# jfjlaros/HUMID

Hardware: AMD Instinct MI355X
Metric: reads/sec deduplicated, 10M PE150 UMI=8 d=1 (higher is better)
Workload: dtype u64; 1 GPU; 10000000 reads/GPU x 1 GPU (one shuffled read set of 10000000 reads, sliced by input order), PE150 UMI=8 in header -> 24-nt packed words (8+8+8), d=1, directional clustering; synthetic molecules=N/4, family 1+Geom(3), p_sub=1e-3, p_N=1e-4; reads_per_gpu=10000000, word_nt=24, distance=1, method=directional

## Files before the change

humid_amd/_lib.py:

```python
from __future__ import annotations

import ctypes as C
import os

_HERE = os.path.dirname(os.path.abspath(__file__))
SO_PATH = os.path.join(_HERE, "libhumid_hip.so")

u64p = C.POINTER(C.c_uint64)
u32p = C.POINTER(C.c_uint32)
u8p = C.POINTER(C.c_uint8)


class HumidSummary(C.Structure):
    _fields_ = [("total", C.c_uint64), ("usable", C.c_uint64), ("unique", C.c_uint64),
                ("clusters", C.c_uint64), ("edges", C.c_uint64), ("nonsingle", C.c_uint64),
                ("ms_count", C.c_float), ("ms_neighbours", C.c_float), ("ms_cluster", C.c_float),
                ("ms_map", C.c_float), ("ms_total", C.c_float), ("ms_h2d", C.c_float),
                ("ms_d2h", C.c_float), ("ms_k_insert", C.c_float), ("ms_k_pairs", C.c_float),
                ("ms_k_cluster", C.c_float), ("ms_k_map", C.c_float), ("ms_k_part", C.c_float),
                ("ms_k_unperm", C.c_float), ("count_mode_used", C.c_uint32)]

    def asdict(self):
        d = {k: getattr(self, k) for k, _ in self._fields_}
        d["records8"] = bool(d["count_mode_used"] >> 8)
# ... 208 lines not shown
    "humid_stage_count": (C.c_int, [C.c_void_p, C.c_void_p, C.c_void_p, C.c_uint64, C.c_uint32,
                                    C.c_uint64, C.c_uint64, C.c_uint64, u64p, u64p]),
    "humid_stage_unique": (C.c_int, [C.c_void_p, C.POINTER(C.c_void_p), C.POINTER(C.c_void_p),
                                     C.POINTER(C.c_void_p)]),
    "humid_stage_graph": (C.c_int, [C.c_void_p, C.c_void_p, C.c_void_p, C.c_uint64, C.c_uint32,
                                    C.c_uint32, C.c_uint32, C.POINTER(C.c_void_p),
                                    C.POINTER(C.c_void_p), C.POINTER(HumidSummary)]),
    "humid_stage_map": (C.c_int, [C.c_void_p, C.c_void_p, C.c_void_p, C.c_uint64, C.c_void_p,
                                  C.c_void_p]),
    "humid_stage_count_dense": (C.c_int, [C.c_void_p, C.c_void_p, C.c_void_p, C.c_uint64, C.c_uint32,
                                          C.c_uint64, C.c_uint64, u64p, C.c_uint32, u64p, u64p, u64p]),
    "humid_stage_map_dense": (C.c_int, [C.c_void_p, C.c_void_p, C.c_void_p, C.POINTER(C.c_void_p), u64p]),
    "humid_stage_pairs": (C.c_int, [C.c_void_p, C.c_void_p, C.c_uint64, C.c_uint32, C.c_uint32,
                                    C.c_uint32, C.c_uint32, C.POINTER(C.c_void_p), u64p]),
    "humid_graph_split_info": (C.c_int, [C.c_void_p, C.POINTER(C.c_uint64), C.POINTER(C.c_uint64), u32p]),
    "humid_get_run_roads": (C.c_int, [C.c_void_p, C.POINTER(HumidRunRoads)]),
    "humid_stage_kernel_ms": (C.c_int, [C.c_void_p, C.POINTER(C.c_float), C.POINTER(C.c_float), u32p]),
    "humid_stage_route_words": (C.c_int, [C.c_void_p, C.c_void_p, C.c_uint64, C.POINTER(C.c_void_p)]),
    "humid_stage_route": (C.c_int, [C.c_void_p, C.c_void_p, C.c_void_p, C.c_uint64, u64p, u64p, C.c_uint32, u64p,
                                    C.POINTER(C.c_void_p), C.POINTER(C.c_void_p)]),
    "humid_stage_route_check": (C.c_int, [C.c_void_p]),
    "humid_stage_exchange_ids": (C.c_int, [C.c_void_p, C.c_void_p, C.c_void_p, C.c_void_p, C.c_uint64,
                                           C.c_uint64, C.c_uint64, C.c_uint64, C.POINTER(C.c_void_p),
                                           C.POINTER(C.c_void_p)]),
    "humid_stage_plan_info": (C.c_int, [C.c_void_p, C.c_uint32, C.c_uint32, C.c_uint64, u32p, u32p]),
    "humid_stage_combo_route": (C.c_int, [C.c_void_p, C.c_void_p, C.c_void_p, C.c_uint64, C.c_uint64,
                                          C.c_uint32, C.c_uint32, C.c_uint64, C.c_uint32, C.c_uint32,
                                          C.POINTER(C.c_void_p), u64p]),
    "humid_stage_pairs_keyed": (C.c_int, [C.c_void_p, C.c_void_p, C.c_uint64, C.c_int, C.c_uint64,
                                          C.c_void_p, C.c_uint32, C.c_uint32, C.c_uint64, C.c_uint32,
# ... 66 lines not shown
```

humid_amd/api.py:

```python
from __future__ import annotations

import ctypes as C

import numpy as np

from . import _lib

DIRECTIONAL = 0
MAXIMUM = 1

BEST_LEAF, BEST_CLUSTER = 0, 1
NO_READ = 0xffffffff
NO_TILE = 0xffffffff
_BEST_SCOPES = {"leaf": BEST_LEAF, "cluster": BEST_CLUSTER, BEST_LEAF: BEST_LEAF, BEST_CLUSTER: BEST_CLUSTER}

STRAND_TOP, STRAND_BOTTOM, STRAND_NONE = 0, 1, 2

BC_FILTERED, BC_EXACT, BC_CORRECTED, BC_AMBIGUOUS, BC_UNMATCHED = range(5)

CELLS_TOP, CELLS_EXPECTED, CELLS_MIN_READS = 0, 1, 2


class HumidError(RuntimeError):
    def __init__(self, code, msg):
# ... 616 lines not shown
        self._check(self._lib.humid_get_leaves(self._h, _vp(out["word"]), _vp(out["count"]),
                                               _vp(out["first_read"]), _vp(out["degree"]),
                                               _vp(out["cluster_id"]), _vp(out["is_max_leaf"])))
        if getattr(self, "_grouped_summary", None) is self.summary:
            out["group"] = np.zeros(u, np.uint32)
            self._check(self._lib.humid_get_leaf_groups(self._h, _vp(out["group"])))
        if getattr(self, "_keyed_summary", None) is self.summary:
            out["key"] = self.group_keys()[out["group"]] if u else np.zeros(0, np.uint64)
        return out

    def graph_split_info(self):
        a, b, f = C.c_uint64(), C.c_uint64(), C.c_uint32()
        self._check(self._lib.humid_graph_split_info(self._h, C.byref(a), C.byref(b), C.byref(f)))
        return dict(pairs_direct=a.value, pairs_graph=b.value, full_graph_built=f.value)

    def run_roads(self):
        r = _lib.HumidRunRoads()
        self._check(self._lib.humid_get_run_roads(self._h, C.byref(r)))
        return r.asdict()

    def adjacency(self):
        u = int(self.summary["unique"])
        e2 = 2 * int(self.summary["edges"])
        off = np.zeros(u + 1, np.uint32)
        idx = np.zeros(max(e2, 1), np.uint32)
        self._check(self._lib.humid_get_adjacency(self._h, _vp(off), _vp(idx)))
        return off, idx[:e2]

    def clusters(self):
        c = int(self.summary["clusters"])
# ... 218 lines not shown
```

humid_amd/csrc/humid_hip.hip:

```cpp
#include "pipeline.hip.h"
#include "passes.hip.h"

static std::string g_err;
extern "C" __attribute__((visibility("hidden"))) void humid_set_global_error(const char *text) { g_err = text ? text : ""; }

extern "C" {

uint32_t humid_abi_version(void) { return HUMID_ABI_VERSION; }

int humid_device_count(void) {
  int n = 0;
  if (hipGetDeviceCount(&n) != hipSuccess) return 0;
  return n;
}

const char *humid_last_error(const humid_ctx *ctx) { return ctx ? ctx->err.c_str() : g_err.c_str(); }

int humid_ctx_create(humid_ctx **out, int device, void *stream) {
  humid_ctx *c = nullptr;
  if (!out) return fail(nullptr, HUMID_E_INVALID, "out is null");
  *out = nullptr;
  int ndev = 0;
  hipError_t e = hipGetDeviceCount(&ndev);
  if (e != hipSuccess || ndev == 0)
// ... 142 lines not shown
  }
  if (strcmp(key, "compact_graph") == 0) {
    c->use_compact = value != 0;
    return HUMID_OK;
  }
  if (strcmp(key, "group_buckets") == 0) {
    c->group_buckets = value != 0;
    return HUMID_OK;
  }
  if (strcmp(key, "fused_search") == 0) {
    c->fused_search = value != 0;
    return HUMID_OK;
  }
  if (strcmp(key, "pair_split") == 0) {
    c->pair_split = value != 0;
    return HUMID_OK;
  }
  if (strcmp(key, "padded_partition") == 0) {
    c->pt_padded = value != 0;
    return HUMID_OK;
  }
  if (strcmp(key, "force_comm") == 0) {
    c->force_comm = value != 0;
    return HUMID_OK;
  }
  if (strcmp(key, "bucket_walk") == 0) {
    if (value < 0 || value > (1 << 24)) return fail(c, HUMID_E_INVALID, "bucket_walk must be 0 (no limit) .. 2^24");
    c->walk_max = (u32)value;
    return HUMID_OK;
  }
// ... 231 lines not shown
#define NEED_LEAVES()                                                                         \
  do {                                                                                        \
    if (!c) return fail(nullptr, HUMID_E_INVALID, "ctx is null");                             \
    if (!state_has_leaves(c)) return fail(c, HUMID_E_STATE, "no completed dedup run / graph stage in this context"); \
    HIPCHK(hipSetDevice(c->device));                                                          \
    TRY(expand_compact(c));                                                                   \
  } while (0)

int humid_graph_split_info(humid_ctx *c, uint64_t *pairs_direct, uint64_t *pairs_graph, uint32_t *full_graph_built) {
  if (!c) return fail(nullptr, HUMID_E_INVALID, "ctx is null");
  if (!state_has_leaves(c)) return fail(c, HUMID_E_STATE, "no completed dedup run / graph stage in this context");
  const bool split = c->cg_valid && c->cg_split;
  if (pairs_direct) *pairs_direct = split ? c->cg_iso : 0;
  if (pairs_graph) *pairs_graph = split ? c->cg_R : c->E;
  if (full_graph_built) *full_graph_built = (!split || c->cg_full) ? 1u : 0u;
  return HUMID_OK;
}

int humid_get_run_roads(humid_ctx *c, humid_run_roads *out) {
  if (!c) return fail(nullptr, HUMID_E_INVALID, "ctx is null");
  if (!out) return fail(c, HUMID_E_INVALID, "null argument");
  if (c->state.holds == CtxState::NOTHING) return fail(c, HUMID_E_STATE, "no completed run or stage call in this context");
  *out = c->roads;
  return HUMID_OK;
}

int humid_get_leaves(humid_ctx *c, uint64_t *word, uint32_t *count, uint32_t *first_read,
                     uint32_t *degree, uint32_t *cluster_id, uint8_t *is_max_leaf) {
  NEED_LEAVES();
  size_t U = (size_t)c->gU;
// ... 1167 lines not shown
```

humid_amd/csrc/kernels_cgraph.hip.h:

```cpp
#ifndef HUMID_KERNELS_CGRAPH_HIP_H
#define HUMID_KERNELS_CGRAPH_HIP_H

#include "common.hip.h"
#include "kernels_graph.hip.h"
#include "kernels_cluster.hip.h"

#define ER_REGIONS 64u
#define ER_STRIDE 32u
struct EdgeRegs {
  u64 *e;
  u32 cap_r;
  u32 *cur;
  const u64 *far;
  u32 n_far;
};
__device__ __forceinline__ u32 er_count(const EdgeRegs &er, u32 r) {
  if (r == ER_REGIONS) return er.n_far;
  const u32 c = er.cur[r * ER_STRIDE];
  return c < er.cap_r ? c : er.cap_r;
}
__device__ __forceinline__ u64 *er_at(const EdgeRegs &er, u32 r, u32 k) {
  return r == ER_REGIONS ? (u64 *)er.far + k : er.e + (size_t)r * er.cap_r + k;
}

// ... 190 lines not shown
  if (PASS0) pa_emit<PA_PPT, 4, MULTI>(word, IdxSelf{}, i0, 256u, n, found, first_off, rule, er, bits, multi, overflow, lds);
  else pa_emit<PA_PPT, 4, MULTI>(word, IdxGlobal{V}, i0, 256u, n, found, first_off, rule, er, bits, multi, overflow, lds);
  PH(2); PH(3); PH(4);
  PH_END(5, 4, (blockIdx.x & 15u) == 5u);
}

struct WordsLds {
  const u64 *sw;
  __device__ __forceinline__ u64 operator()(u32 j) const { return sw[j]; }
};
struct IdxGrouped {
  const unsigned short *inv;
  const u32 *v_in;
  __device__ __forceinline__ u32 operator()(u32 j) const { return v_in[inv[j]]; }
};
template <bool MULTI>
struct PairSearchDevT {
  static constexpr bool on = true;
  PairRule<u64> rule;
  EdgeRegs er;
  u32 *bits;
  u32 *multi;
  ull *big;
  u32 *overflow;
  template <u32 NP, u32 T>
  __device__ __forceinline__ void in_bin(const u64 *sw, u32 n, const unsigned short *inv, const u32 *v_in, u32 *scratch) const {
    const WordsLds word{sw};
    u32 found[NP], first_off[NP];
#pragma unroll
    for (u32 q = 0; q < NP; q++) {
      const u32 i = threadIdx.x + q * T;
      found[q] = 0; first_off[q] = 0;
      if (i < n) pa_walk(word, sw[i], sw[i + 1 < n ? i + 1 : i], i, n, rule, big, found[q], first_off[q]);
    }
    pa_emit<NP, T / 64u, MULTI>(word, IdxGrouped{inv, v_in}, threadIdx.x, T, n, found, first_off, rule, er, bits, multi, overflow, scratch);
  }
};

using PairSearchDev = PairSearchDevT<false>;

static __global__ void __launch_bounds__(256)
k_mark_pairs(const u64 *__restrict__ pairs, u32 n_pairs, u32 n_leaves, u32 *bits, u32 *bad, u32 *multi = nullptr) {
  HUMID_GUARD_LAST_VGPR();
  const u32 k = blockIdx.x * blockDim.x + threadIdx.x;
  if (k >= n_pairs) return;
  const u64 e = pairs[k];
  const u32 a = (u32)(e >> 32), b = (u32)e;
  if (a >= n_leaves || b >= n_leaves || a == b) { *bad = 1; return; }
  if (multi) { mark_end<true>(bits, multi, a); mark_end<true>(bits, multi, b); }
  else { mark_end<false>(bits, multi, a); mark_end<false>(bits, multi, b); }
// ... 343 lines not shown
```

humid_amd/csrc/kernels_graph.hip.h:

```cpp
#ifndef HUMID_KERNELS_GRAPH_HIP_H
#define HUMID_KERNELS_GRAPH_HIP_H

#include "common.hip.h"

#define MAX_COMBOS 20
#define MAX_FIELDS 8
struct ComboPlan {
  u32 ncombo;
  u32 key_bits;
  W2 mask[MAX_COMBOS];
  u8 nfield[MAX_COMBOS];
  u8 shift[MAX_COMBOS][MAX_FIELDS];
  u8 width[MAX_COMBOS][MAX_FIELDS];
};

template <class WT>
struct EarlierMasksT {
  WT m[MAX_COMBOS];
};

struct ComboFields {
  u32 nf;
  u8 shift[MAX_FIELDS];
  u8 width[MAX_FIELDS];
// ... 42 lines not shown
  u32 kb;
  __device__ __forceinline__ bool load(u32 j, u64 &payload) const {
    const W2 w = words[j];
    u64 k = 0;
#pragma unroll
    for (u32 f = 0; f < MAX_FIELDS; f++) {
      if (f < cf.nf) {
        const u32 wd = cf.width[f];
        k = ((wd >= 64) ? 0ull : (k << wd)) | w_field(w, cf.shift[f], wd);
      }
    }
    payload = k << (64 - kb);
    return true;
  }
  __device__ __forceinline__ u64 key(u64 payload) const { return payload; }
};

__device__ __forceinline__ u32 uf_find(const u32 *P, u32 x) {
  u32 p = ld_agent(&P[x]);
  while (p != x) { x = p; p = ld_agent(&P[x]); }
  return x;
}

__device__ __forceinline__ void uf_union(u32 *P, u32 a, u32 b) {
  while (true) {
    a = uf_find(P, a);
    b = uf_find(P, b);
    if (a == b) return;
    if (a > b) { u32 t = a; a = b; b = t; }
    if (atomicCAS(&P[b], b, a) == b) return;
// ... 613 lines not shown
```

humid_amd/csrc/kernels_part.hip.h:

```cpp
#ifndef HUMID_KERNELS_PART_HIP_H
#define HUMID_KERNELS_PART_HIP_H

#include "common.hip.h"
#include "kernels_count.hip.h"

#define PT_THREADS 1024u
#define PT_TILE 8192u
#define PT_IPT (PT_TILE / PT_THREADS)
#define PT_MAXBINS 512u
#define PT_MAXBINS1 1024u

struct PtInput {
  const u64 *words;
  const u8 *filtered;
  u64 rlo, rhi;
  u32 check_range;
  PartKeyOp key;
};
__device__ __forceinline__ bool pt_load(const PtInput &in, u32 r, u64 &key) {
  if (in.filtered && in.filtered[r]) return false;
  const u64 w = in.words[r];
  if (in.check_range && (w < in.rlo || w > in.rhi)) return false;
  key = in.key(w);
  return true;
// ... 219 lines not shown
  for (u32 b = threadIdx.x; b < nb; b += PT_THREADS) h[b] = 0;
  __syncthreads();
  const u32 beg = s_beg, n = s_cnt;
  for (u32 j = threadIdx.x; j < n; j += PT_THREADS)
    atomicAdd(&h[(u32)(src.key(k_in[beg + j]) >> (64 - d1 - d2)) & (nb - 1)], 1u);
  __syncthreads();
  for (u32 b = threadIdx.x; b < nb; b += PT_THREADS)
    if (h[b]) atomicAdd(&hist_fine[(s_c << d2) | b], h[b]);
}

struct NoSearch { static constexpr bool on = false; };
#define GF_THREADS 1024u
#define GF_MAXBITS 15u
#define GF_SMALL 7872u
#define GF_MID 32768u
template <class SRC, int SIZE, class SEARCH = NoSearch>
__global__ void __launch_bounds__(GF_THREADS, SIZE == 0 ? 8 : 4)
k_group_fine(SRC src, const u64 *__restrict__ k_in, const u32 *__restrict__ v_in, const u32 *__restrict__ cbase, u32 d1,
             u32 d2, u64 *__restrict__ k_out, u32 *__restrict__ v_out, u32 cap1, SEARCH srch = SEARCH()) {
  HUMID_GUARD_LAST_VGPR();
  static_assert(SIZE == 0 || !SEARCH::on, "the search rides in the launch of the small bins");
  static_assert(GF_SMALL * 2u + 32u <= (1u << (GF_MAXBITS - 1)), "the grouped words and the emit's words fit the counter area");
  constexpr bool BIG = SIZE == 2;
  constexpr u32 INV_WORDS = SIZE == 0 ? GF_SMALL / 2u + 16u : (1u << (GF_MAXBITS - 1)) + 16u;
  __shared__ __attribute__((aligned(8))) u32 gf_lds[BIG ? (1u << GF_MAXBITS) + 16 : (1u << (GF_MAXBITS - 1)) + INV_WORDS];
  const u32 nb = 1u << d2, c = blockIdx.x;
  PH_DECL;
  PH(0);
  const u32 beg = cbase[c], end = cbase[c + 1];
  if (beg >= end) return;
// ... 23 lines not shown
#pragma unroll
      for (u32 q = 0; q < GF_RPT; q++) {
        const u32 j = threadIdx.x + q * GF_THREADS;
        ff[q] = fine(kk[q]);
        if (j < n) atomicAdd(&gf_lds[ff[q] >> 1], 1u << (16 * (ff[q] & 1)));
      }
    } else {
      for (u32 j = threadIdx.x; j < n; j += GF_THREADS) {
        const u32 f = fine(k_in[j]);
        atomicAdd(&gf_lds[f >> 1], 1u << (16 * (f & 1)));
      }
    }
    PH(2);
    __syncthreads();
    PH(3);
    const u32 words = nb >= 2 ? nb / 2 : 1u;
    const u32 n_waves = GF_THREADS / 64u;
    const u32 per_wave = (words + n_waves - 1) / n_waves, wbeg = wv * per_wave, wend = wbeg + per_wave < words ? wbeg + per_wave : words;
    u32 tot = 0;
    for (u32 w = wbeg + lane; w < wend; w += 64) { const u32 x = gf_lds[w]; tot += (x & 0xffffu) + (x >> 16); }
#pragma unroll
    for (u32 dd = 32; dd; dd >>= 1) tot += __shfl_xor(tot, dd);
    if (lane == 0) wsum[wv] = tot;
    __syncthreads();
    u32 run = 0;
    for (u32 q = 0; q < wv; q++) run += wsum[q];
    for (u32 w0 = wbeg; w0 < wend; w0 += 64) {
      const u32 w = w0 + lane;
      const u32 x = w < wend ? gf_lds[w] : 0u;
      const u32 mine = (x & 0xffffu) + (x >> 16);
      const u32 incl = wave_incl_scan(mine);
      const u32 lo = run + incl - mine, hi = lo + (x & 0xffffu);
      if (w < wend) gf_lds[w] = lo | (hi << 16);
      run += (u32)__builtin_amdgcn_readlane((int)incl, 63);
    }
    __syncthreads();
    PH(4);
    if constexpr (SIZE == 0) {
      u32 oldq[GF_RPT];
#pragma unroll
      for (u32 q = 0; q < GF_RPT; q++) {
        const u32 j = threadIdx.x + q * GF_THREADS;
        oldq[q] = j < n ? atomicAdd(&gf_lds[ff[q] >> 1], 1u << (16 * (ff[q] & 1))) : 0u;
      }
#pragma unroll
      for (u32 q = 0; q < GF_RPT; q++) {
        const u32 j = threadIdx.x + q * GF_THREADS;
        if (j < n) inv[(oldq[q] >> (16 * (ff[q] & 1))) & 0xffffu] = (unsigned short)j;
      }
      PH(5);
      __syncthreads();
// ... 58 lines not shown
  u32 run = incl - mine;
  for (u32 q = 0; q < wv; q++) run += wsum[q];
  if (b0 < nb)
    for (u32 q = 0; q < per; q++) {
      const u32 x = gf_lds[b0 + q];
      gf_lds[b0 + q] = run;
      run += x;
    }
  __syncthreads();
  for (u32 j = threadIdx.x; j < n; j += GF_THREADS) {
    const u64 w = k_in[j];
    const u32 p = atomicAdd(&gf_lds[fine(w)], 1u);
    k_out[p] = w;
    v_out[p] = v_in[j];
  }
}

#define UW_MAXBINS 2048u
#define UW_MAXSHIFT 15u

static __global__ void __launch_bounds__(1024)
k_unperm_bins(const u32 *__restrict__ vals, const u32 *__restrict__ pslot, const u64 *__restrict__ slot_out,
              const u32 *__restrict__ n_pos_dev, u32 n_pos_max, u32 n_reads, u32 wshift, u32 n_bins, u32 *ucur,
              u64 *__restrict__ rec) {
  HUMID_GUARD_LAST_VGPR();
  __shared__ u64 srec[PT_TILE];
  __shared__ unsigned short sbin[PT_TILE];
  __shared__ u32 cnt[UW_MAXBINS], loff[UW_MAXBINS + 1], goff[UW_MAXBINS], wsum[16];
  u32 n_pos = n_pos_dev ? *n_pos_dev : n_pos_max;
  if (n_pos > n_pos_max) n_pos = n_pos_max;
// ... 114 lines not shown
```

humid_amd/csrc/kernels_part8.hip.h:

```cpp
#ifndef HUMID_KERNELS_PART8_HIP_H
#define HUMID_KERNELS_PART8_HIP_H

#include "common.hip.h"
#include "kernels_count.hip.h"
#include "kernels_part.hip.h"

#define P8_CAP2_LOG 10u
#define P8_CAP2 (1u << P8_CAP2_LOG)
#define P8_RPT (P8_CAP2 / 256u)

struct RecKey {
  u64 lo, scale;
  u32 z, kbits;
  u32 pow2;
  __host__ __device__ __forceinline__ u64 operator()(u64 w) const { return ((w - lo) * scale) >> z; }
  __device__ __forceinline__ u64 word(u64 k) const {
    if (pow2) return lo + k;
    const u64 x = k << z, q = x / scale;
    return lo + q + ((x - q * scale) ? 1u : 0u);
  }
};

struct Reads8 {
  const u64 *words;
// ... 18 lines not shown
    const u32 bin = b0 + sub;
    if (bin >= nb) continue;
    const u32 beg = loff[bin], n = loff[bin + 1] - beg;
    for (u32 k = gl; k < n; k += G) {
      const u64 d = dst(bin, k);
      if (d != ~0ull) out[d] = srec[beg + k];
    }
  }
}
__device__ __forceinline__ u32 p8_group(u32 records, u32 nb) {
  u32 g = 8;
  while (g < 64 && g * nb < records) g <<= 1;
  return g;
}

template <class SRC, u32 THREADS>
__global__ void __launch_bounds__(THREADS)
k_p8_scatter1(SRC src, u32 n_reads, u32 kbits, u32 d1, u32 ibits, u32 cap1, u32 *cursor, u64 *__restrict__ out, ull *ctr) {
  HUMID_GUARD_LAST_VGPR();
  constexpr u32 TILE = THREADS * PT_IPT;
  __shared__ u64 srec[TILE];
  __shared__ u32 cnt[PT_MAXBINS1], loff[PT_MAXBINS1 + 1], goff[PT_MAXBINS1], wsum[16];
  const u32 nb = 1u << d1;
  PH_DECL;
  PH(0);
  const u32 t_beg = blockIdx.x * TILE;
  const u32 t_cnt = (t_beg >= n_reads) ? 0u : ((n_reads - t_beg < TILE) ? n_reads - t_beg : TILE);
  for (u32 b = threadIdx.x; b < nb; b += THREADS) cnt[b] = 0;
  __syncthreads();
  PH(1);
  const u32 rbits = kbits - d1;
// ... 7 lines not shown
    if (j < t_cnt && src.load(t_beg + j, k)) {
      const u32 bin = (u32)(k >> rbits);
      rec[q] = ((k & ((1ull << rbits) - 1ull)) << ibits) | (u64)(t_beg + j);
      binrank[q] = bin << 16 | atomicAdd(&cnt[bin], 1u);
    }
  }
  PH(2);
  __syncthreads();
  PH(3);
  block_exscan_1024(cnt, loff, nb, wsum);
  PH(4);
  if (threadIdx.x < nb) {
    const u32 c = cnt[threadIdx.x];
    const u32 had = c ? atomicAdd(&cursor[threadIdx.x], c) : 0u;
    goff[threadIdx.x] = threadIdx.x * cap1 + (had < cap1 ? had : cap1);
    if (had + c > cap1) ctr[CTR_SPECIAL] = 1;
  }
  PH(5);
#pragma unroll
  for (u32 q = 0; q < PT_IPT; q++)
    if (binrank[q] != NONE32) srec[loff[binrank[q] >> 16] + (binrank[q] & 0xffffu)] = rec[q];
  __syncthreads();
  PH(6);
  p8_write_bins(srec, loff, nb, p8_group(loff[nb], nb), out,
                [&](u32 bin, u32 k) -> u64 { return goff[bin] + k < (bin + 1) * cap1 ? (u64)goff[bin] + k : ~0ull; });
  PH(7);
  PH_END(1, 7, (blockIdx.x & 15u) == 3u);
}

static __global__ void __launch_bounds__(1024, 8)
k_p8_scatter2(const u64 *__restrict__ in, const u32 *__restrict__ tprefix, const u32 *__restrict__ cbase, u32 kbits, u32 d1,
// ... 552 lines not shown
```

humid_amd/csrc/pipeline.hip.h:

```cpp
#ifndef HUMID_PIPELINE_HIP_H
#define HUMID_PIPELINE_HIP_H

#include <fcntl.h>
#include <sys/mman.h>
#include <sys/stat.h>
#include <unistd.h>

#include <atomic>
#include <cerrno>
#include <chrono>
#include <type_traits>
#include <utility>

#include "common.hip.h"
#include "prims.hip.h"
#include "kernels_count.hip.h"
#include "kernels_part.hip.h"
#include "kernels_part8.hip.h"
#include "kernels_graph.hip.h"
#include "kernels_cluster.hip.h"
#include "kernels_cgraph.hip.h"
#include "kernels_map.hip.h"
#include "kernels_xchg.hip.h"
#include "kernels_wide.hip.h"
// ... 125 lines not shown
  u64 cg_pairs_bound = 0;
  u32 cg_method = 0;
  const u32 *ctr_x[3] = {nullptr, nullptr, nullptr};
  DBuf xo_gw, xo_gc;
  DBuf xo_regs, xo_inv;
  u64 xr_ecap = 0;
  DBuf xo_send, xo_int, xo_cross, xo_sel, xo_selall, xo_parent, xo_flag, xo_xroot, xo_xcbits, xo_xcblk, xo_xcid, xo_xcall, xo_ldeg, xo_cnt;
  DBuf pw_a, pw_ai, pw_b, pw_bi;
  DBuf p8_a, p8_b, p8_cur, p8_status;
  bool use_rec8 = true;
  bool last_rec8 = false;
  const u32 *rec_cursor2 = nullptr;
  DBuf pt_work, unperm_rec, route_tiles;
  bool group_buckets = true;
  bool fused_search = true;
  bool pt_padded = true;
  bool use_tile_partition = true;
  bool last_part_tiled = false;
  int x_test_fail_after = -1, x_gathers = 0;
  bool x_hist_done = false, x_peer_failed = false;
  bool route_checked = true;
  const u32 *route_bad = nullptr;
  bool last_unperm_tiled = false;
  bool oc_valid = false, oc_fits = false;
  u32 oc_n = 0, oc_nt = 0;
  u64 oc_lo = 0, oc_scale = 0;
  u32 n_parts = 0;
  bool stage_map_timed = false;
  bool last_count_sorted = false;
  u32 g_wpr = 1;
// ... 1009 lines not shown
  if (n_runs) HIPCHK(hipMemcpy(d_runs, runs.data(), (size_t)n_runs * sizeof(BigRun), hipMemcpyHostToDevice));
  *d_runs_out = d_runs;
  return HUMID_OK;
}

static ComboFields plan_fields(const ComboPlan &plan, u32 cb) {
  ComboFields cf;
  cf.nf = plan.nfield[cb];
  for (u32 f = 0; f < MAX_FIELDS; f++) { cf.shift[f] = plan.shift[cb][f]; cf.width[f] = plan.width[cb][f]; }
  return cf;
}
struct GroupRide {
  PairSearchDev group;
  bool did_group = false;
  hipEvent_t ev_group[2] = {nullptr, nullptr};
};
static void group_fine_with_search(humid_ctx *c, const FieldsSrc &src, const u64 *k0, const u32 *v0, const u32 *cbase, u32 d1, u32 d2, u64 *ws,
                                   u32 *vs, u32 cap1, const PairSearchDev &s);
template <class SRC, class WT>
static int group_words_by_stretch(humid_ctx *c, const ComboPlan &plan, u32 cb, const WT *W, u32 n, u64 *ws, u32 *vs, bool *done,
                                  bool may_pad = false, GroupRide *ride = nullptr) {
  hipStream_t st = c->stream;
  u32 bit_n = 0;
  for (u32 f = 0; f < plan.nfield[cb]; f++) bit_n += plan.width[cb][f];
  *done = c->group_buckets && plan.nfield[cb] >= 1 && bit_n >= 2 && bit_n <= 24 && n >= 4096;
  c->gf_valid = nullptr;
  if (!*done) return HUMID_OK;
  const u32 d1 = bit_n >= 18 ? 9u : (bit_n + 1) / 2, d2 = bit_n - d1;
  const u32 nb1 = 1u << d1;
  const bool padded = may_pad && c->gf_padded;
  const u32 cap1 = padded ? n / nb1 + n / nb1 / 4 + 1024 : 0u;
  const size_t room = padded ? (size_t)nb1 * cap1 : (size_t)n;
  ENSURE(c->pt_work, (size_t)(1024 + 513 + 513 + 516) * 4);
  u32 *hist1 = c->pt_work.as<u32>(), *cursor1 = hist1 + 512, *cbase = cursor1 + 512, *tprefix = cbase + 513, *dummy = tprefix + 513;
  if (padded) {
    if (!c->gf_cur.p) {
      ENSURE(c->gf_cur, 512 * 4);
      HIPCHK(hipMemsetAsync(c->gf_cur.p, 0, 512 * 4, st));
    }
    cursor1 = c->gf_cur.as<u32>();
  } else HIPCHK(hipMemsetAsync(c->pt_work.p, 0, 1024 * 4, st));
  ENSURE(c->seg_k0, room * 8);
  ENSURE(c->seg_v0, room * 4);
  const SRC src{W, plan_fields(plan, cb), bit_n};
  const u32 tiles1 = (n + PT_TILE - 1) / PT_TILE;
  if (!padded) {
    hipLaunchKernelGGL(k_pt_hist1<SRC>, dim3(tiles1 < 512 ? tiles1 : 512), dim3(1024), 0, st, src, n, d1, hist1);
    hipLaunchKernelGGL(k_pt_scan1, dim3(1), dim3(1024), 0, st, (const u32 *)hist1, d1, 0u, cbase, tprefix, dummy, dummy + 513, 0u);
  }
  static const bool gs_small = getenv("HUMID_GS_THREADS") ? atoi(getenv("HUMID_GS_THREADS")) == 512 : false;
  const bool ride_ok = ride && std::is_same<SRC, FieldsSrc>::value && padded && cap1 <= GF_SMALL;
  if (gs_small)
    hipLaunchKernelGGL((k_pt_scatter<1, SRC, 512>), dim3((n + 4095) / 4096), dim3(512), 0, st, src, n, (const u64 *)nullptr,
                       (const u32 *)nullptr, (const u32 *)nullptr, (const u32 *)nullptr, d1, d2, (const u32 *)cbase, cursor1,
                       c->seg_k0.as<u64>(), c->seg_v0.as<u32>(), (u32 *)nullptr, cap1, &c->d_ctr[CTR_GOVER]);
  else
    hipLaunchKernelGGL((k_pt_scatter<1, SRC>), dim3(tiles1), dim3(1024), 0, st, src, n, (const u64 *)nullptr,
                       (const u32 *)nullptr, (const u32 *)nullptr, (const u32 *)nullptr, d1, d2, (const u32 *)cbase, cursor1,
                       c->seg_k0.as<u64>(), c->seg_v0.as<u32>(), (u32 *)nullptr, cap1, &c->d_ctr[CTR_GOVER]);
  if (padded)
    hipLaunchKernelGGL(k_pt_scan1, dim3(1), dim3(1024), 0, st, (const u32 *)cursor1, d1, 0u, cbase, tprefix, dummy, dummy + 513, cap1, cursor1);
  c->gf_valid = padded ? (const u32 *)(cbase + nb1) : (const u32 *)nullptr;
  const u32 largest = padded ? cap1 : n;
  if (ride_ok) {
    if constexpr (std::is_same<SRC, FieldsSrc>::value) {
      if (ride->ev_group[0]) HIPCHK(hipEventRecord(ride->ev_group[0], st));
// ... 166 lines not shown
  else
    hipLaunchKernelGGL((k_pairs_append<true, WT>), grid, blk, 0, c->stream, w.W, w.V, w.n, rule, er, bits, multi, big, overflow, n_valid);
}
static PairSearchDev pairs_append_dev(const PairSearch<u64> &s, u64 mask, u32 cb, const EdgeRegs &er, u32 *bits, u32 *multi, ull *big,
                                      u32 *overflow) {
  return PairSearchDev{PairRule<u64>{mask, s.em, cb, s.distance, s.walk_max}, er, bits, multi, big, overflow};
}
static void group_fine_with_search(humid_ctx *c, const FieldsSrc &src, const u64 *k0, const u32 *v0, const u32 *cbase, u32 d1, u32 d2, u64 *ws,
                                   u32 *vs, u32 cap1, const PairSearchDev &s) {
  if (s.multi)
    hipLaunchKernelGGL((k_group_fine<FieldsSrc, 0, PairSearchDevT<true>>), dim3(1u << d1), dim3(GF_THREADS), 0, c->stream, src, k0, v0, cbase, d1, d2,
                       ws, vs, cap1, PairSearchDevT<true>{s.rule, s.er, s.bits, s.multi, s.big, s.overflow});
  else
    hipLaunchKernelGGL((k_group_fine<FieldsSrc, 0, PairSearchDev>), dim3(1u << d1), dim3(GF_THREADS), 0, c->stream, src, k0, v0, cbase, d1, d2, ws,
                       vs, cap1, s);
}
static void comp_stats(humid_ctx *c, u32 U) {
  hipLaunchKernelGGL(k_comp_stats, dim3(blocks_for(U)), dim3(256), 0, c->stream, c->deg.as<u32>(), c->parent.as<u32>(), U, c->csize.as<u32>());
  hipLaunchKernelGGL(k_comp_count, dim3(512), dim3(256), 0, c->stream, c->deg.as<u32>(), c->parent.as<u32>(), c->csize.as<u32>(), U, c->d_ctr,
                     c->small_roots.as<u32>());
}

template <class WT>
static int stage_graph(humid_ctx *c, const WT *g_word, const u32 *g_cnt, u32 U, u32 word_nt,
                       u32 distance, u32 method, humid_summary &s, u32 &n_pair_segs_out,
                       const u64 *ext_edges = nullptr, u64 n_ext_edges = 0) {
  hipStream_t st = c->stream;
  c->g_word = g_word;
  c->g_wpr = (u32)(sizeof(WT) / 8);
  c->g_cnt = g_cnt;
// ... 227 lines not shown
}

template <class WT>
static int stage_graph_compact(humid_ctx *c, const WT *g_word, const u32 *g_cnt, u32 U, u32 word_nt,
                               u32 distance, u32 method, humid_summary &s, u32 &n_pair_segs_out,
                               const u64 *ext_edges = nullptr, u64 n_ext_edges = 0) {
  hipStream_t st = c->stream;
  c->g_word = g_word;
  c->g_wpr = (u32)(sizeof(WT) / 8);
  c->g_cnt = g_cnt;
  c->gU = U;
  c->cg_valid = false;
  c->cg_expanded = false;
  c->cg_split = c->cg_full = c->cg_m_late = c->cg_broken = false;
  c->cg_iso = c->cg_R = 0;
  const bool split = c->pair_split;
  const ComboPlan plan = make_plan(word_nt - c->gk_nt, distance, U, c->force_segments, true, c->gk_nt);
  const PairSearch<WT> ps = pair_search<WT>(c, plan, distance);
  const bool given = ext_edges != nullptr;
  const bool search = !given && distance > 0 && U > 1;
  if (search && plan.ncombo == 1 && plan.key_bits == 0 && U > (1u << 18))
    return fail(c, HUMID_E_OVERFLOW, "distance %u over %u-nt words compares all pairs of %u unique words: too many neighbour pairs",
                distance, word_nt, U);
  if (given && n_ext_edges > 0x7fffffffull) return fail(c, HUMID_E_OVERFLOW, "too many neighbour pairs");
  const u32 nseg = search ? plan.ncombo : 0;
  const u32 n_words = (((U + 31) / 32) + 7) & ~7u, n_blk = n_words / 8;
  c->cg_nblocks = n_blk;
  ENSURE(c->cg_bits, (size_t)n_words * 4);
  ENSURE(c->cg_nbits, (size_t)n_words * 4);
  ENSURE(c->cg_blk, ((size_t)n_blk + 1) * 4);
// ... 39 lines not shown
      if (split) {
        z.p[4] = multi; z.n[4] = n_words;
        z.p[5] = c->cg_rbits.as<u32>(); z.n[5] = n_words;
        z.p[6] = c->small.as<u32>(); z.n[6] = SPLIT_WORDS;
      }
      hipLaunchKernelGGL(k_zero_many, dim3(64), dim3(256), 0, st, z);
    }
    auto search_alone = [&](u32 seg) -> int {
      if (seg < 8 && c->kev_on) HIPCHK(hipEventRecord(c->kev[20 + 2 * seg], st));
      pairs_append<WT>(c, ps, walked_seg<WT>(c, plan, seg, g_word, U), er, c->cg_bits.as<u32>(), multi, &c->d_ctr[CTR_BIGMASK],
                       (u32 *)&c->d_ctr[CTR_EOVER], seg_valid[seg]);
      if (seg < 8 && c->kev_on) HIPCHK(hipEventRecord(c->kev[21 + 2 * seg], st));
      return HUMID_OK;
    };
    const bool ride_on = c->fused_search && std::is_same<WT, u64>::value;
    for (u32 seg = 0; seg < nseg; seg++) {
      bool searched = false;
      if (seg) {
        seg_valid[seg] = nullptr;
        if (!ordered_seg[seg]) {
          GroupRide ride;
          if constexpr (std::is_same<WT, u64>::value) {
            if (ride_on) {
              ride.group = pairs_append_dev(ps, w_from<u64>(plan.mask[seg]), seg, er, c->cg_bits.as<u32>(), multi, &c->d_ctr[CTR_BIGMASK], (u32 *)&c->d_ctr[CTR_EOVER]);
              if (seg < 8 && c->kev_on) { ride.ev_group[0] = c->kev[20 + 2 * seg]; ride.ev_group[1] = c->kev[21 + 2 * seg]; }
            }
          }
          TRY(bucket_order<WT>(c, plan, seg, g_word, U, seg_ws<WT>(c, seg, U), seg_vs(c, seg, U), true, ride_on ? &ride : nullptr));
          seg_valid[seg] = c->gf_valid;
          searched = ride.did_group;
        }
        ordered_seg[seg] = true;
      }
      if (!searched) TRY(search_alone(seg));
    }
    if (n_far)
      hipLaunchKernelGGL(k_mark_pairs, dim3(blocks_for(n_far)), dim3(256), 0, st, far, (u32)n_far, U, c->cg_bits.as<u32>(), bad, multi);
    if (split) {
      const u64 rest_cap = (u64)ER_REGIONS * er.cap_r + n_far;
      if (rest_cap > 0x7fffffffull) return fail(c, HUMID_E_OVERFLOW, "too many neighbour pairs");
      ENSURE(c->cg_rest, (size_t)(rest_cap + 1) * 8);
      const u32 gx = (u32)std::min<u64>(std::max<u64>(blocks_for(std::max<u64>(er.cap_r, er.n_far), SPLIT_PPT * 256), 1), 4096);
      u32 *sp = c->small.as<u32>();
      if (method == HUMID_METHOD_MAXIMUM)
        hipLaunchKernelGGL(k_pairs_split<true>, dim3(gx, ER_REGIONS + 1), dim3(256), 0, st, er, (const u32 *)multi, g_cnt, c->cg_pres.as<u32>(),
                           c->cg_nbits.as<u32>(), c->cg_rbits.as<u32>(), c->cg_rest.as<u64>(), (u32)rest_cap, U, sp);
      else
// ... 29 lines not shown
      continue;
    }
    if (given) {
      u32 h_bad = 0;
      HIPCHK(hipMemcpyAsync(&h_bad, bad, 4, hipMemcpyDeviceToHost, st));
      HIPCHK(hipStreamSynchronize(st));
      if (h_bad) return fail(c, HUMID_E_INVALID, "malformed edge list (node index out of range)");
    }
    if (search && cgs.big_mask && !far) {
      const u64 big_mask = cgs.big_mask;
      u64 got = 0;
      for (int phase = 0; phase < 2; phase++) {
        u64 at = 0;
        for (u32 seg = 0; seg < nseg; seg++) {
          if (!(big_mask >> seg & 1)) continue;
          const Walked<WT> w = walked_seg<WT>(c, plan, seg, g_word, U);
          std::vector<BigRun> runs;
          const BigRun *d_runs = nullptr;
          TRY(find_big_runs<WT>(c, w.W, U, w.mask, ps.walk_max, seg, runs, &d_runs));
          if (!runs.back().tile0) continue;
          const ull start = phase ? at : 0;
          HIPCHK(hipMemcpyAsync(&c->d_ctr[CTR_SPECIAL], &start, sizeof(ull), hipMemcpyHostToDevice, st));
          HIPCHK(hipStreamSynchronize(st));
          tiles_emit<WT>(c, ps, w, d_runs, runs, phase ? PM_EMIT_FILL : PM_EMIT_COUNT,
                         EmitSink{nullptr, nullptr, c->cg_far.as<u64>(), &c->d_ctr[CTR_SPECIAL]});
          HIPCHK(hipGetLastError());
          TRY(read_counters(c));
          if (phase == 0) got += c->h_ctr[CTR_SPECIAL]; else at = c->h_ctr[CTR_SPECIAL];
        }
        if (phase == 0) {
// ... 1239 lines not shown
```

include/humid_hip.h:

```cpp
#ifndef HUMID_HIP_H
#define HUMID_HIP_H

#include <stddef.h>
#include <stdint.h>

#ifdef __cplusplus
extern "C" {
#endif

#define HUMID_OK             0
#define HUMID_E_INVALID     -1
#define HUMID_E_UNSUPPORTED -2
#define HUMID_E_NOMEM       -3
#define HUMID_E_HIP         -4
#define HUMID_E_OVERFLOW    -5
#define HUMID_E_STATE       -6

#define HUMID_METHOD_DIRECTIONAL 0u
#define HUMID_METHOD_MAXIMUM     1u

#define HUMID_ABI_VERSION 5u

typedef struct humid_ctx humid_ctx;

// ... 318 lines not shown
                             const uint64_t **d_unique_edges, uint64_t *n_unique_edges);

int humid_stage_owned_results(humid_ctx *ctx, const uint32_t *d_local_cluster_id,
                              const uint8_t *d_local_is_max, const uint64_t *shard_begin,
                              uint32_t n_shards, const uint32_t **d_packed, uint64_t *counts);
int humid_stage_owner_perm(humid_ctx *ctx, const uint64_t *d_words, const uint8_t *d_filtered,
                           uint64_t n_reads, const uint64_t *range_lo, const uint64_t *range_hi,
                           uint32_t n_ranks, const uint32_t **d_perm, uint64_t *counts);
int humid_stage_owner_perm_wide(humid_ctx *ctx, const uint64_t *d_words, const uint8_t *d_filtered,
                                uint64_t n_reads, uint32_t word_nt, const uint64_t *range_lo, const uint64_t *range_hi,
                                uint32_t n_ranks, const uint32_t **d_perm, uint64_t *counts);
int humid_stage_scatter(humid_ctx *ctx, const uint32_t *d_perm, const uint32_t *d_packed,
                        uint64_t n_recv, uint64_t n_reads, uint32_t *d_cluster_id, uint8_t *d_keep);

int humid_graph_split_info(humid_ctx *ctx, uint64_t *pairs_direct, uint64_t *pairs_graph, uint32_t *full_graph_built);
#define HUMID_ROAD_PART_PADDED_REDO 1
#define HUMID_ROAD_ORDERS_REDONE    2
#define HUMID_ROAD_REGIONS_REGROWN  3
#define HUMID_ROAD_FAR_TILES        4
#define HUMID_ROAD_CSR_TILES        5
#define HUMID_ROAD_JOIN_PIECES      6
#define HUMID_ROADS_MAX 32
typedef struct humid_run_roads {
  uint32_t n_events;
  uint32_t graph_attempts;
  uint8_t events[HUMID_ROADS_MAX];
} humid_run_roads;
int humid_get_run_roads(humid_ctx *ctx, humid_run_roads *out);
int humid_stage_kernel_ms(humid_ctx *ctx, float *ms_k_insert, float *ms_k_map, uint32_t *count_mode_used);
int humid_stage_route_words(humid_ctx *ctx, const uint64_t *d_words, uint64_t n_send,
// ... 58 lines not shown
```

Baseline: 17.72 billion reads/s.

## Search neighbour pairs on packed records and skip storing segment orders

```diff
diff --git a/humid_amd/_lib.py b/humid_amd/_lib.py
--- a/humid_amd/_lib.py
+++ b/humid_amd/_lib.py
@@ -246,6 +246,7 @@
     "humid_stage_pairs": (C.c_int, [C.c_void_p, C.c_void_p, C.c_uint64, C.c_uint32, C.c_uint32,
                                     C.c_uint32, C.c_uint32, C.POINTER(C.c_void_p), u64p]),
     "humid_graph_split_info": (C.c_int, [C.c_void_p, C.POINTER(C.c_uint64), C.POINTER(C.c_uint64), u32p]),
+    "humid_group_records_info": (C.c_int, [C.c_void_p, u32p, u32p]),
     "humid_get_run_roads": (C.c_int, [C.c_void_p, C.POINTER(HumidRunRoads)]),
     "humid_stage_kernel_ms": (C.c_int, [C.c_void_p, C.POINTER(C.c_float), C.POINTER(C.c_float), u32p]),
     "humid_stage_route_words": (C.c_int, [C.c_void_p, C.c_void_p, C.c_uint64, C.POINTER(C.c_void_p)]),
diff --git a/humid_amd/api.py b/humid_amd/api.py
--- a/humid_amd/api.py
+++ b/humid_amd/api.py
@@ -654,6 +654,11 @@
         self._check(self._lib.humid_graph_split_info(self._h, C.byref(a), C.byref(b), C.byref(f)))
         return dict(pairs_direct=a.value, pairs_graph=b.value, full_graph_built=f.value)
 
+    def group_records_info(self):
+        a, b = C.c_uint32(), C.c_uint32()
+        self._check(self._lib.humid_group_records_info(self._h, C.byref(a), C.byref(b)))
+        return dict(searched_on_records=a.value, orders_stored=b.value)
+
     def run_roads(self):
         r = _lib.HumidRunRoads()
         self._check(self._lib.humid_get_run_roads(self._h, C.byref(r)))
diff --git a/humid_amd/csrc/humid_hip.hip b/humid_amd/csrc/humid_hip.hip
--- a/humid_amd/csrc/humid_hip.hip
+++ b/humid_amd/csrc/humid_hip.hip
@@ -180,6 +180,10 @@
   }
   if (strcmp(key, "pair_split") == 0) {
     c->pair_split = value != 0;
+    return HUMID_OK;
+  }
+  if (strcmp(key, "group_records") == 0) {
+    c->group_records = value != 0;
     return HUMID_OK;
   }
   if (strcmp(key, "padded_partition") == 0) {
@@ -441,6 +445,14 @@
   if (pairs_direct) *pairs_direct = split ? c->cg_iso : 0;
   if (pairs_graph) *pairs_graph = split ? c->cg_R : c->E;
   if (full_graph_built) *full_graph_built = (!split || c->cg_full) ? 1u : 0u;
+  return HUMID_OK;
+}
+
+int humid_group_records_info(humid_ctx *c, uint32_t *searched_on_records, uint32_t *orders_stored) {
+  if (!c) return fail(nullptr, HUMID_E_INVALID, "ctx is null");
+  if (!state_has_leaves(c)) return fail(c, HUMID_E_STATE, "no completed dedup run / graph stage in this context");
+  if (searched_on_records) *searched_on_records = c->cg_valid ? c->gr_rides : 0u;
+  if (orders_stored) *orders_stored = c->cg_valid ? c->gr_orders : 0u;
   return HUMID_OK;
 }
 
diff --git a/humid_amd/csrc/kernels_cgraph.hip.h b/humid_amd/csrc/kernels_cgraph.hip.h
--- a/humid_amd/csrc/kernels_cgraph.hip.h
+++ b/humid_amd/csrc/kernels_cgraph.hip.h
@@ -228,6 +228,12 @@
   const u32 *v_in;
   __device__ __forceinline__ u32 operator()(u32 j) const { return v_in[inv[j]]; }
 };
+struct IdxRecords {
+  const unsigned short *inv;
+  const u64 *recs;
+  u32 ibits;
+  __device__ __forceinline__ u32 operator()(u32 j) const { return (u32)(recs[inv[j]] & ((1ull << ibits) - 1ull)); }
+};
 template <bool MULTI>
 struct PairSearchDevT {
   static constexpr bool on = true;
@@ -239,6 +245,14 @@
   u32 *overflow;
   template <u32 NP, u32 T>
   __device__ __forceinline__ void in_bin(const u64 *sw, u32 n, const unsigned short *inv, const u32 *v_in, u32 *scratch) const {
+    walk_bin<NP, T>(sw, n, IdxGrouped{inv, v_in}, scratch);
+  }
+  template <u32 NP, u32 T>
+  __device__ __forceinline__ void in_bin_recs(const u64 *sw, u32 n, const unsigned short *inv, const u64 *recs, u32 ibits, u32 *scratch) const {
+    walk_bin<NP, T>(sw, n, IdxRecords{inv, recs, ibits}, scratch);
+  }
+  template <u32 NP, u32 T, class IDX>
+  __device__ __forceinline__ void walk_bin(const u64 *sw, u32 n, const IDX &idx, u32 *scratch) const {
     const WordsLds word{sw};
     u32 found[NP], first_off[NP];
 #pragma unroll
@@ -247,7 +261,7 @@
       found[q] = 0; first_off[q] = 0;
       if (i < n) pa_walk(word, sw[i], sw[i + 1 < n ? i + 1 : i], i, n, rule, big, found[q], first_off[q]);
     }
-    pa_emit<NP, T / 64u, MULTI>(word, IdxGrouped{inv, v_in}, threadIdx.x, T, n, found, first_off, rule, er, bits, multi, overflow, scratch);
+    pa_emit<NP, T / 64u, MULTI>(word, idx, threadIdx.x, T, n, found, first_off, rule, er, bits, multi, overflow, scratch);
   }
 };
 
diff --git a/humid_amd/csrc/kernels_graph.hip.h b/humid_amd/csrc/kernels_graph.hip.h
--- a/humid_amd/csrc/kernels_graph.hip.h
+++ b/humid_amd/csrc/kernels_graph.hip.h
@@ -80,6 +80,24 @@
     return true;
   }
   __device__ __forceinline__ u64 key(u64 payload) const { return payload; }
+};
+
+struct RecSqueeze {
+  u32 p, d1;
+  __device__ __forceinline__ u64 low(u64 x) const { return x & ((1ull << p) - 1ull); }
+  __device__ __forceinline__ u32 bin(u64 w) const { return (u32)(w >> p) & ((1u << d1) - 1u); }
+  __device__ __forceinline__ u64 squeeze(u64 w) const { return (w >> p >> d1 << p) | low(w); }
+  __device__ __forceinline__ u64 word(u32 c, u64 s) const { return (s >> p << p << d1) | ((u64)c << p) | low(s); }
+};
+struct FieldsRecs {
+  const u64 *words;
+  RecSqueeze sq;
+  u32 rbits;
+  __device__ __forceinline__ bool load(u32 j, u64 &k) const {
+    const u64 w = words[j];
+    k = ((u64)sq.bin(w) << rbits) | (sq.squeeze(w) & ((1ull << rbits) - 1ull));
+    return true;
+  }
 };
 
 __device__ __forceinline__ u32 uf_find(const u32 *P, u32 x) {
diff --git a/humid_amd/csrc/kernels_part.hip.h b/humid_amd/csrc/kernels_part.hip.h
--- a/humid_amd/csrc/kernels_part.hip.h
+++ b/humid_amd/csrc/kernels_part.hip.h
@@ -257,6 +257,31 @@
 #define GF_MAXBITS 15u
 #define GF_SMALL 7872u
 #define GF_MID 32768u
+__device__ __forceinline__ void gf_scan16(u32 *cnt, u32 *wsum, u32 nb) {
+  const u32 lane = threadIdx.x & 63, wv = threadIdx.x >> 6;
+  const u32 words = nb >= 2 ? nb / 2 : 1u;
+  const u32 n_waves = GF_THREADS / 64u;
+  const u32 per_wave = (words + n_waves - 1) / n_waves, wbeg = wv * per_wave, wend = wbeg + per_wave < words ? wbeg + per_wave : words;
+  u32 tot = 0;
+  for (u32 w = wbeg + lane; w < wend; w += 64) { const u32 x = cnt[w]; tot += (x & 0xffffu) + (x >> 16); }
+#pragma unroll
+  for (u32 dd = 32; dd; dd >>= 1) tot += __shfl_xor(tot, dd);
+  if (lane == 0) wsum[wv] = tot;
+  __syncthreads();
+  u32 run = 0;
+  for (u32 q = 0; q < wv; q++) run += wsum[q];
+  for (u32 w0 = wbeg; w0 < wend; w0 += 64) {
+    const u32 w = w0 + lane;
+    const u32 x = w < wend ? cnt[w] : 0u;
+    const u32 mine = (x & 0xffffu) + (x >> 16);
+    const u32 incl = wave_incl_scan(mine);
+    const u32 lo = run + incl - mine, hi = lo + (x & 0xffffu);
+    if (w < wend) cnt[w] = lo | (hi << 16);
+    run += (u32)__builtin_amdgcn_readlane((int)incl, 63);
+  }
+  __syncthreads();
+}
+
 template <class SRC, int SIZE, class SEARCH = NoSearch>
 __global__ void __launch_bounds__(GF_THREADS, SIZE == 0 ? 8 : 4)
 k_group_fine(SRC src, const u64 *__restrict__ k_in, const u32 *__restrict__ v_in, const u32 *__restrict__ cbase, u32 d1,
@@ -310,27 +335,7 @@
     PH(2);
     __syncthreads();
     PH(3);
-    const u32 words = nb >= 2 ? nb / 2 : 1u;
-    const u32 n_waves = GF_THREADS / 64u;
-    const u32 per_wave = (words + n_waves - 1) / n_waves, wbeg = wv * per_wave, wend = wbeg + per_wave < words ? wbeg + per_wave : words;
-    u32 tot = 0;
-    for (u32 w = wbeg + lane; w < wend; w += 64) { const u32 x = gf_lds[w]; tot += (x & 0xffffu) + (x >> 16); }
-#pragma unroll
-    for (u32 dd = 32; dd; dd >>= 1) tot += __shfl_xor(tot, dd);
-    if (lane == 0) wsum[wv] = tot;
-    __syncthreads();
-    u32 run = 0;
-    for (u32 q = 0; q < wv; q++) run += wsum[q];
-    for (u32 w0 = wbeg; w0 < wend; w0 += 64) {
-      const u32 w = w0 + lane;
-      const u32 x = w < wend ? gf_lds[w] : 0u;
-      const u32 mine = (x & 0xffffu) + (x >> 16);
-      const u32 incl = wave_incl_scan(mine);
-      const u32 lo = run + incl - mine, hi = lo + (x & 0xffffu);
-      if (w < wend) gf_lds[w] = lo | (hi << 16);
-      run += (u32)__builtin_amdgcn_readlane((int)incl, 63);
-    }
-    __syncthreads();
+    gf_scan16(gf_lds, wsum, nb);
     PH(4);
     if constexpr (SIZE == 0) {
       u32 oldq[GF_RPT];
@@ -419,6 +424,65 @@
     k_out[p] = w;
     v_out[p] = v_in[j];
   }
+}
+
+template <class SRC, class SQ, class SEARCH>
+__global__ void __launch_bounds__(GF_THREADS, 8)
+k_group_fine_recs(SRC src, SQ sq, const u64 *__restrict__ recs, u32 *cursor, u32 d1, u32 d2, u32 ibits, u32 cap1, SEARCH srch) {
+  HUMID_GUARD_LAST_VGPR();
+  constexpr u32 INV_WORDS = GF_SMALL / 2u + 16u;
+  constexpr u32 GF_RPT = 8;
+  static_assert(GF_RPT * GF_THREADS >= GF_SMALL, "a thread holds its share of a full bin");
+  static_assert(GF_SMALL * 2u + 32u <= (1u << (GF_MAXBITS - 1)), "the grouped words and the emit's words fit the counter area");
+  __shared__ __attribute__((aligned(8))) u32 gf_lds[(1u << (GF_MAXBITS - 1)) + INV_WORDS];
+  const u32 nb = 1u << d2, c = blockIdx.x;
+  u32 n = cursor[c];
+  if (n == 0) return;
+  if (n > cap1) n = cap1;
+  if (n > GF_SMALL) n = GF_SMALL;
+  recs += (size_t)c * cap1;
+  u32 *wsum = gf_lds + (1u << (GF_MAXBITS - 1)) + INV_WORDS - 16;
+  unsigned short *inv = (unsigned short *)(gf_lds + (1u << (GF_MAXBITS - 1)));
+  u64 kk[GF_RPT];
+  u32 ff[GF_RPT];
+#pragma unroll
+  for (u32 q = 0; q < GF_RPT; q++) {
+    const u32 j = threadIdx.x + q * GF_THREADS;
+    kk[q] = j < n ? recs[j] : 0ull;
+  }
+  for (u32 b = threadIdx.x; b < (1u << (GF_MAXBITS - 1)); b += GF_THREADS) gf_lds[b] = 0;
+  __syncthreads();
+  if (threadIdx.x == 0) cursor[c] = 0;
+#pragma unroll
+  for (u32 q = 0; q < GF_RPT; q++) {
+    const u32 j = threadIdx.x + q * GF_THREADS;
+    kk[q] = sq.word(c, kk[q] >> ibits);
+    ff[q] = (u32)(src.key(kk[q]) >> (64 - d1 - d2)) & (nb - 1);
+    if (j < n) atomicAdd(&gf_lds[ff[q] >> 1], 1u << (16 * (ff[q] & 1)));
+  }
+  __syncthreads();
+  gf_scan16(gf_lds, wsum, nb);
+  u32 oldq[GF_RPT];
+#pragma unroll
+  for (u32 q = 0; q < GF_RPT; q++) {
+    const u32 j = threadIdx.x + q * GF_THREADS;
+    oldq[q] = j < n ? atomicAdd(&gf_lds[ff[q] >> 1], 1u << (16 * (ff[q] & 1))) : 0u;
+  }
+#pragma unroll
+  for (u32 q = 0; q < GF_RPT; q++) {
+    const u32 j = threadIdx.x + q * GF_THREADS;
+    oldq[q] = (oldq[q] >> (16 * (ff[q] & 1))) & 0xffffu;
+    if (j < n) inv[oldq[q]] = (unsigned short)j;
+  }
+  __syncthreads();
+  u64 *sw = (u64 *)gf_lds;
+#pragma unroll
+  for (u32 q = 0; q < GF_RPT; q++) {
+    const u32 j = threadIdx.x + q * GF_THREADS;
+    if (j < n) sw[oldq[q]] = kk[q];
+  }
+  __syncthreads();
+  srch.template in_bin_recs<GF_RPT, GF_THREADS>(sw, n, inv, recs, ibits, gf_lds + 2u * GF_SMALL);
 }
 
 #define UW_MAXBINS 2048u
diff --git a/humid_amd/csrc/kernels_part8.hip.h b/humid_amd/csrc/kernels_part8.hip.h
--- a/humid_amd/csrc/kernels_part8.hip.h
+++ b/humid_amd/csrc/kernels_part8.hip.h
@@ -56,7 +56,7 @@
   return g;
 }
 
-template <class SRC, u32 THREADS>
+template <class SRC, u32 THREADS, int OVER = CTR_SPECIAL>
 __global__ void __launch_bounds__(THREADS)
 k_p8_scatter1(SRC src, u32 n_reads, u32 kbits, u32 d1, u32 ibits, u32 cap1, u32 *cursor, u64 *__restrict__ out, ull *ctr) {
   HUMID_GUARD_LAST_VGPR();
@@ -94,7 +94,7 @@
     const u32 c = cnt[threadIdx.x];
     const u32 had = c ? atomicAdd(&cursor[threadIdx.x], c) : 0u;
     goff[threadIdx.x] = threadIdx.x * cap1 + (had < cap1 ? had : cap1);
-    if (had + c > cap1) ctr[CTR_SPECIAL] = 1;
+    if (had + c > cap1) ctr[OVER] = 1;
   }
   PH(5);
 #pragma unroll
diff --git a/humid_amd/csrc/pipeline.hip.h b/humid_amd/csrc/pipeline.hip.h
--- a/humid_amd/csrc/pipeline.hip.h
+++ b/humid_amd/csrc/pipeline.hip.h
@@ -163,6 +163,8 @@
   DBuf pt_work, unperm_rec, route_tiles;
   bool group_buckets = true;
   bool fused_search = true;
+  bool group_records = true;
+  u32 gr_rides = 0, gr_orders = 0;
   bool pt_padded = true;
   bool use_tile_partition = true;
   bool last_part_tiled = false;
@@ -1202,7 +1204,11 @@
   PairSearchDev group;
   bool did_group = false;
   hipEvent_t ev_group[2] = {nullptr, nullptr};
+  u32 word_bits = 0;
+  bool no_order = false;
 };
+static void group_fine_recs_with_search(humid_ctx *c, const FieldsSrc &src, const RecSqueeze &sq, const u64 *recs, u32 *cursor, u32 d1, u32 d2,
+                                        u32 ibits, u32 cap1, const PairSearchDev &s);
 static void group_fine_with_search(humid_ctx *c, const FieldsSrc &src, const u64 *k0, const u32 *v0, const u32 *cbase, u32 d1, u32 d2, u64 *ws,
                                    u32 *vs, u32 cap1, const PairSearchDev &s);
 template <class SRC, class WT>
@@ -1219,25 +1225,43 @@
   const bool padded = may_pad && c->gf_padded;
   const u32 cap1 = padded ? n / nb1 + n / nb1 / 4 + 1024 : 0u;
   const size_t room = padded ? (size_t)nb1 * cap1 : (size_t)n;
-  ENSURE(c->pt_work, (size_t)(1024 + 513 + 513 + 516) * 4);
-  u32 *hist1 = c->pt_work.as<u32>(), *cursor1 = hist1 + 512, *cbase = cursor1 + 512, *tprefix = cbase + 513, *dummy = tprefix + 513;
+  const SRC src{W, plan_fields(plan, cb), bit_n};
+  const u32 tiles1 = (n + PT_TILE - 1) / PT_TILE;
+  u32 *cursor1 = nullptr;
   if (padded) {
     if (!c->gf_cur.p) {
       ENSURE(c->gf_cur, 512 * 4);
       HIPCHK(hipMemsetAsync(c->gf_cur.p, 0, 512 * 4, st));
     }
     cursor1 = c->gf_cur.as<u32>();
-  } else HIPCHK(hipMemsetAsync(c->pt_work.p, 0, 1024 * 4, st));
+  }
   ENSURE(c->seg_k0, room * 8);
+  const bool ride_ok = ride && std::is_same<SRC, FieldsSrc>::value && padded && cap1 <= GF_SMALL;
+  if constexpr (std::is_same<SRC, FieldsSrc>::value) {
+    const u32 ibits = bits_for(n), wb = ride_ok ? ride->word_bits : 0u;
+    if (ride_ok && c->group_records && wb && plan.width[cb][0] >= d1 && wb - d1 + ibits <= 64) {
+      const RecSqueeze sq{(u32)plan.shift[cb][0] + plan.width[cb][0] - d1, d1};
+      const FieldsRecs rsrc{W, sq, wb - d1};
+      hipLaunchKernelGGL((k_p8_scatter1<FieldsRecs, 1024, CTR_GOVER>), dim3(tiles1), dim3(1024), 0, st, rsrc, n, wb, d1, ibits, cap1, cursor1,
+                         c->seg_k0.as<u64>(), c->d_ctr);
+      if (ride->ev_group[0]) HIPCHK(hipEventRecord(ride->ev_group[0], st));
+      group_fine_recs_with_search(c, src, sq, c->seg_k0.as<u64>(), cursor1, d1, d2, ibits, cap1, ride->group);
+      if (ride->ev_group[1]) HIPCHK(hipEventRecord(ride->ev_group[1], st));
+      ride->did_group = ride->no_order = true;
+      HIPCHK(hipGetLastError());
+      return HUMID_OK;
+    }
+  }
   ENSURE(c->seg_v0, room * 4);
-  const SRC src{W, plan_fields(plan, cb), bit_n};
-  const u32 tiles1 = (n + PT_TILE - 1) / PT_TILE;
+  ENSURE(c->pt_work, (size_t)(1024 + 513 + 513 + 516) * 4);
+  u32 *hist1 = c->pt_work.as<u32>(), *cbase = hist1 + 1024, *tprefix = cbase + 513, *dummy = tprefix + 513;
   if (!padded) {
+    cursor1 = hist1 + 512;
+    HIPCHK(hipMemsetAsync(c->pt_work.p, 0, 1024 * 4, st));
     hipLaunchKernelGGL(k_pt_hist1<SRC>, dim3(tiles1 < 512 ? tiles1 : 512), dim3(1024), 0, st, src, n, d1, hist1);
     hipLaunchKernelGGL(k_pt_scan1, dim3(1), dim3(1024), 0, st, (const u32 *)hist1, d1, 0u, cbase, tprefix, dummy, dummy + 513, 0u);
   }
   static const bool gs_small = getenv("HUMID_GS_THREADS") ? atoi(getenv("HUMID_GS_THREADS")) == 512 : false;
-  const bool ride_ok = ride && std::is_same<SRC, FieldsSrc>::value && padded && cap1 <= GF_SMALL;
   if (gs_small)
     hipLaunchKernelGGL((k_pt_scatter<1, SRC, 512>), dim3((n + 4095) / 4096), dim3(512), 0, st, src, n, (const u64 *)nullptr,
                        (const u32 *)nullptr, (const u32 *)nullptr, (const u32 *)nullptr, d1, d2, (const u32 *)cbase, cursor1,
@@ -1434,6 +1458,15 @@
   else
     hipLaunchKernelGGL((k_group_fine<FieldsSrc, 0, PairSearchDev>), dim3(1u << d1), dim3(GF_THREADS), 0, c->stream, src, k0, v0, cbase, d1, d2, ws,
                        vs, cap1, s);
+}
+static void group_fine_recs_with_search(humid_ctx *c, const FieldsSrc &src, const RecSqueeze &sq, const u64 *recs, u32 *cursor, u32 d1, u32 d2,
+                                        u32 ibits, u32 cap1, const PairSearchDev &s) {
+  if (s.multi)
+    hipLaunchKernelGGL((k_group_fine_recs<FieldsSrc, RecSqueeze, PairSearchDevT<true>>), dim3(1u << d1), dim3(GF_THREADS), 0, c->stream, src, sq, recs,
+                       cursor, d1, d2, ibits, cap1, PairSearchDevT<true>{s.rule, s.er, s.bits, s.multi, s.big, s.overflow});
+  else
+    hipLaunchKernelGGL((k_group_fine_recs<FieldsSrc, RecSqueeze, PairSearchDev>), dim3(1u << d1), dim3(GF_THREADS), 0, c->stream, src, sq, recs, cursor,
+                       d1, d2, ibits, cap1, s);
 }
 static void comp_stats(humid_ctx *c, u32 U) {
   hipLaunchKernelGGL(k_comp_stats, dim3(blocks_for(U)), dim3(256), 0, c->stream, c->deg.as<u32>(), c->parent.as<u32>(), U, c->csize.as<u32>());
@@ -1691,6 +1724,7 @@
   c->cg_expanded = false;
   c->cg_split = c->cg_full = c->cg_m_late = c->cg_broken = false;
   c->cg_iso = c->cg_R = 0;
+  c->gr_rides = c->gr_orders = 0;
   const bool split = c->pair_split;
   const ComboPlan plan = make_plan(word_nt - c->gk_nt, distance, U, c->force_segments, true, c->gk_nt);
   const PairSearch<WT> ps = pair_search<WT>(c, plan, distance);
@@ -1760,6 +1794,7 @@
       return HUMID_OK;
     };
     const bool ride_on = c->fused_search && std::is_same<WT, u64>::value;
+    const bool ride_now = ride_on && attempt == 0;
     for (u32 seg = 0; seg < nseg; seg++) {
       bool searched = false;
       if (seg) {
@@ -1767,16 +1802,18 @@
         if (!ordered_seg[seg]) {
           GroupRide ride;
           if constexpr (std::is_same<WT, u64>::value) {
-            if (ride_on) {
+            if (ride_now) {
               ride.group = pairs_append_dev(ps, w_from<u64>(plan.mask[seg]), seg, er, c->cg_bits.as<u32>(), multi, &c->d_ctr[CTR_BIGMASK], (u32 *)&c->d_ctr[CTR_EOVER]);
               if (seg < 8 && c->kev_on) { ride.ev_group[0] = c->kev[20 + 2 * seg]; ride.ev_group[1] = c->kev[21 + 2 * seg]; }
+              ride.word_bits = word_nt <= 32 ? 2 * word_nt : 0u;
             }
           }
-          TRY(bucket_order<WT>(c, plan, seg, g_word, U, seg_ws<WT>(c, seg, U), seg_vs(c, seg, U), true, ride_on ? &ride : nullptr));
+          TRY(bucket_order<WT>(c, plan, seg, g_word, U, seg_ws<WT>(c, seg, U), seg_vs(c, seg, U), true, ride_now ? &ride : nullptr));
           seg_valid[seg] = c->gf_valid;
           searched = ride.did_group;
+          ordered_seg[seg] = !ride.no_order;
+          if (ride.no_order) c->gr_rides++; else c->gr_orders++;
         }
-        ordered_seg[seg] = true;
       }
       if (!searched) TRY(search_alone(seg));
     }
@@ -1836,6 +1873,11 @@
         u64 at = 0;
         for (u32 seg = 0; seg < nseg; seg++) {
           if (!(big_mask >> seg & 1)) continue;
+          if (seg && !ordered_seg[seg]) {
+            TRY(bucket_order<WT>(c, plan, seg, g_word, U, seg_ws<WT>(c, seg, U), seg_vs(c, seg, U), true));
+            ordered_seg[seg] = true;
+            c->gr_orders++;
+          }
           const Walked<WT> w = walked_seg<WT>(c, plan, seg, g_word, U);
           std::vector<BigRun> runs;
           const BigRun *d_runs = nullptr;
diff --git a/include/humid_hip.h b/include/humid_hip.h
--- a/include/humid_hip.h
+++ b/include/humid_hip.h
@@ -356,6 +356,7 @@
                         uint64_t n_recv, uint64_t n_reads, uint32_t *d_cluster_id, uint8_t *d_keep);
 
 int humid_graph_split_info(humid_ctx *ctx, uint64_t *pairs_direct, uint64_t *pairs_graph, uint32_t *full_graph_built);
+int humid_group_records_info(humid_ctx *ctx, uint32_t *searched_on_records, uint32_t *orders_stored);
 #define HUMID_ROAD_PART_PADDED_REDO 1
 #define HUMID_ROAD_ORDERS_REDONE    2
 #define HUMID_ROAD_REGIONS_REGROWN  3
```

Measured after the change: 18.41 billion reads/s (median of 6 runs). 1.04x the previous value.
